# halixness/distributed-3d-diffusion-pytorch

Measured on AMD Instinct MI355X. Metric: train imgs/sec (whole node), SRN cars 64x64 bs128, higher is better.
Workload: dtype bf16; 1 GPU; model=XUNet ch128 ch_mult(1,2,2,4) 136.7M params (3DiM, reference xunet.py), global_batch=128, seq_len=4096, image_size=64, per_gpu_batch=128, micro_batch=128, hip_graph=False, parallelism=dp1, dist_backend=none, tuned_gemms=True, backend=hip

## Files before the change

### distributed_3d_diffusion_pytorch_amd/ops/_abi.py

```python
from __future__ import annotations

import ctypes as C

P = C.c_void_p
I = C.c_int
L = C.c_long
F = C.c_float
U64 = C.c_ulonglong
IP = C.POINTER(C.c_int)

SIGNATURES = {
    "d3d_gn_plan": [I, I, I, IP, IP],
    "d3d_gn_cfg": [I, I, I],
    "d3d_gn_cfg_small": [I, I],
    "d3d_gn_stats": [P, I, I, I, I, F, P, P, P, I, P],
    "d3d_gn_apply": [P, P, P, P, P, I, I, I, I, I, P],
    "d3d_gn_film": [P, P, P, P, P, P, I, I, I, I, F, U64, I, P, P],
    "d3d_gn_bwd": [I, P, P, P, P, P, P, I, I, I, I, F, U64, P, P, P, P, P, P, P, P],
    "d3d_ray_dir": [P, P, P, P, I, I, I, I, P],
    "d3d_border_fix": [P, P, I, I, I, I, I, I, I, P, P],
    "d3d_border_sums": [P, P, I, I, I, I, P],
    "d3d_gn_apply2": [I, P, P, P, P, P, P, P, I, I, I, I, F, F, U64, I, P, P, I, I, P, P],
    "d3d_set_words64": [P, I, C.c_longlong, C.c_longlong, C.c_longlong, P],
    "d3d_sgemm_jobs": [P, I, I, P],
    "d3d_gn_ab": [P, P, P, P, P, I, I, I, I, F, I, P],
    "d3d_gn_ab_silu": [P, P, P, I, I, I, P],
    "d3d_gn_img_cfg": [I],
    "d3d_gn_img_ok": [I, I, I],
    "d3d_gn_img_ok_n": [I, I, I, I],
    "d3d_gn_img_wide_cfg": [I, I],
    "d3d_gn_img_fwd": [I, P, P, P, P, P, P, I, I, I, I, F, F, U64, I, P, P, I, P, P],
    "d3d_gn_img_bwd": [I, P, P, P, P, P, P, I, I, I, I, F, U64, P, P, P, I, P, P, P, I, P, F, P, F, P],
    "d3d_gn_bwd2": [I, P, P, P, P, P, P, I, I, I, I, F, U64, P, P, P, P, P, P, P, I, I, P, P, P, I, P, F, P, F, P],
    "d3d_conv_s64_cfg": [I],
    "d3d_conv_hsm_cfg": [I],
    "d3d_gemm_small_k": [I],
    "d3d_gemm_mf": [I],
    "d3d_gemm_w8_waves": [I],
    "d3d_attn_bwd_cfg": [I],
    "d3d_attn_fwd_cfg": [I],
    "d3d_colsum_jobs": [P, I, P],
    "d3d_conv_halo_cfg": [I],
    "d3d_period_sum": [P, P, I, L, P],
    "d3d_silu": [P, P, L, P],
    "d3d_dsilu": [P, P, P, L, P],
    "d3d_avgpool2": [P, P, I, I, I, I, I, P],
    "d3d_upsample2": [P, P, I, I, I, I, I, P],
    "d3d_add_scale": [P, P, P, F, L, P],
    "d3d_set_words": [P, I, F, F, F, F, F, F, F, F, P],
    "d3d_add_scale_gn": [P, P, P, F, L, I, I, I, P, P],
    "d3d_sampler_step": [P, P, P, P, P, I, I, F, F, F, F, F, I, U64, I, P],
    "d3d_sampler_inputs": [P, P, I, I, P, P, U64, L, P, P, P],
    "d3d_sampler_step2": [P, P, P, I, I, P, P, U64, L, I, P],
    "d3d_sampler_solve": [P, P, P, P, I, I, P, P, U64, L, I, P],
    "d3d_randn_hash": [P, L, U64, L, P],
    "d3d_diffusion_fwd2": [P, I, I, U64, P, L, F, F, F, P, P, P, P, I, P],
    "d3d_diff_loss": [P, P, I, I, I, I, P, P, P, I, F, P],
    "d3d_diff_loss_bwd": [P, P, P, I, I, I, I, P, P, I, F, P],
    "d3d_adam": [P, P, P, P, P, L, F, F, F, F, F, F, F, F, P],
    "d3d_adam_dev": [P, P, P, P, P, L, P, P],
    "d3d_chansum": [P, P, P, P, I, I, I, I, P],
    "d3d_colsum": [P, L, I, P, P, P, I, P],
    "d3d_conv3_gn_ok": [I, I, I, I, I],
    "d3d_conv3_gn": [P, P, P, P, I, I, I, I, I, I, P, I, IP, P, P],
    "d3d_conv3": [P, P, P, P, P, P, I, I, I, I, I, I, I, I, I, I, I, F, I, I, P, I, P, I, IP, P, IP, P],
    "d3d_conv_plan": [I, I, I, I, I, I],
    "d3d_set_wgrad_impl": [I],
    "d3d_conv_wgrad_plan2": [I, I, I, I, I, I, IP, IP],
    "d3d_conv_wgrad_plan3": [I, I, I, I, I, I, I, I, I, IP, IP],
    "d3d_pack_weight": [P, P, I, I, I, I, I, I, P],
    "d3d_set_conv_impl": [I, P],
    "d3d_pack_all": [P, P, I, P],
    "d3d_conv_wgrad_cat": [P, P, P, I, P, P, P, I, I, I, I, I, I, P],
    "d3d_conv_wgrad_seg": [P, P, P, I, I, I, I, I, I, I, I, I, I, I, I, I, P, P, P, P],
    "d3d_wgrad_scatter": [P, I, I, I, I, P, I, I, P, P, P, P],
    "d3d_conv_wgrad3": [P, P, P, P, P, I, I, I, I, I, I, I, I, I, I, I, I, F, P],
    "d3d_ray_posenc": [P, P, P, P, P, P, P, P, I, I, I, P],
    "d3d_cond_prep": [P, P, P, I, C.c_double, C.c_double, P, P, P, P],
    "d3d_attn_fwd": [P, P, P, I, I, I, I, I, F, P],
    "d3d_adam_fused": [P, P, P, P, P, P, P, P, I, P, P, I, I, P],
    "d3d_mlp_ws": [I, I, I],
    "d3d_mlp_pe": [P, I, I, F, P, P],
    "d3d_mlp_mm": [P, P, I, I, I, I, I, I, P, P, P, P, P],
    "d3d_mlp_wgrad": [P, P, I, I, I, I, P, P, I, P],
    "d3d_gemm": [P, P, P, P, I, P, I, I, I, I, I, I, I, F, F, P, I, I, I, P],
    "d3d_gemm_cat": [P, P, P, I, P, P, I, I, I, I, I, F, F, P],
    "d3d_sgemm_strided": [P, P, P, I, I, I, I, L, L, L, L, L, L, L, L, L, F, F, P],
    "d3d_wgrad_tn_plan": [I, I, L, I, I],
    "d3d_wgrad_tn": [P, P, P, P, I, I, L, I, I, I, P],
    "d3d_wgrad_tn_tune": [I],
    "d3d_gemm_nt_ok": [I, I, I, I, I],
    "d3d_gemm_tune": [I, I, I],
    "d3d_gemm_nt": [P, P, P, P, P, I, I, I, I, I, I, I, F, F, P],
    "d3d_gemm_nt_gn": [P, P, P, P, P, I, I, I, I, I, I, I, F, F, P, I, I, P],
    "d3d_attn_bwd": [P, P, P, P, P, P, I, I, I, I, I, F, P],
    "d3d_attn_bwd_slabs": [I, I, I, I],
    "d3d_wgrad_group_cfg": [I, I, I],
    "d3d_wgrad_group_ok": [P],
    "d3d_wgrad_group_stages": [I],
    "d3d_wgrad_group_halo": [I, I, I],
    "d3d_wgrad_group_halo_big": [I, I],
    "d3d_wgrad_group_halo_pk": [I],
    "d3d_wgrad_group_engine": [P],
    "d3d_wgrad_group": [P, I, P, L, P],
    "d3d_wgrad_group_plan": [P, I, IP, IP, C.POINTER(C.c_long)],
    "d3d_loss_rows_parts": [I],
    "d3d_diff_loss_rows": [P, P, I, I, I, I, P, P, P],
    "d3d_loss_bins": [P, I, P, P, I, I, I, C.c_double, C.c_double, C.c_double, P],
    "d3d_image_metrics": [P, P, I, I, I, I, I, C.POINTER(C.c_double), P, P, P],
}


def declare(lib: C.CDLL) -> None:
    for name, args in SIGNATURES.items():
        fn = getattr(lib, name, None)
        if fn is None:
            continue
        fn.argtypes = args
        fn.restype = C.c_long if name in RET_LONG else C.c_int


RET_LONG = {"d3d_mlp_ws", "d3d_wgrad_group"}
```

### distributed_3d_diffusion_pytorch_amd/ops/csrc/conv.hip

```cpp
#include "common.h"
#include <stdlib.h>

#include <algorithm>

D3D_API int d3d_colsum(const float* in, long R, int Cc, float* part, float* out, float* out_odd, int accumulate,
                       hipStream_t st);

typedef __attribute__((ext_vector_type(4))) short s16x4;
typedef __attribute__((ext_vector_type(8))) short s16x8;
typedef __attribute__((address_space(3))) s16x4 lds_s16x4;

namespace {

template <int TAPS, bool TRANS>
__global__ void __launch_bounds__(256, 2)
conv_glds_k(const bf16* __restrict__ I, const bf16* __restrict__ Wp, const float* __restrict__ bias,
            const float* __restrict__ row_bias, const bf16* __restrict__ res, bf16* __restrict__ O,
            const bf16* __restrict__ zero16, int Nimg, int IH, int IW, int IC, int ICp, int OH, int OW, int OC,
            int ldo, int stride, float scale, int res_nmod, float* __restrict__ part, int korder) {
  constexpr int BM = 128, BN = 128, BKk = 64;
  constexpr int WM = 64, WN = 64, TM = 4, TN = 4;
  constexpr int STAGE = (BM + BN) * BKk;
  __shared__ __attribute__((aligned(16))) bf16 smem[2 * STAGE];
  typedef __attribute__((address_space(3))) void lds_void;
// ... 548 lines not shown
      for (int i = 0; i < TM; ++i)
#pragma unroll
        for (int j = 0; j < TN; ++j)
          acc[i][j] = __builtin_amdgcn_mfma_f32_16x16x32_bf16(af[i], bfr[j], acc[i][j], 0, 0, 0);
    }
    __builtin_amdgcn_s_setprio(0);
    asm volatile("s_waitcnt vmcnt(0) lgkmcnt(0)" ::: "memory");
    __builtin_amdgcn_s_barrier();
  }

  constexpr int NH = WN / 64;
  float gs[TM][NH], gq[TM][NH];
#pragma unroll
  for (int i = 0; i < TM; ++i)
#pragma unroll
    for (int h = 0; h < NH; ++h) gs[i][h] = gq[i][h] = 0.f;
  float cb[TM][4];
#pragma unroll
  for (int i = 0; i < TM; ++i) {
    const int co = m0 + wm * WM + i * 16 + fq * 4;
#pragma unroll
    for (int e = 0; e < 4; ++e) cb[i][e] = (bias && co + e < OC) ? bias[co + e] : 0.f;
  }
#pragma unroll
  for (int j = 0; j < TN; ++j) {
    const long pix = n0 + wn * WN + j * 16 + fr;
    if (pix >= Mpix) continue;
    const int img = (int)(pix / OHW);
    const long rpix = res_nmod > 0 ? (long)(img % res_nmod) * OHW + (pix - (long)img * OHW) : pix;
#pragma unroll
    for (int i = 0; i < TM; ++i) {
      const int co = m0 + wm * WM + i * 16 + fq * 4;
      if (co >= OC) continue;
      float v[4];
#pragma unroll
      for (int e = 0; e < 4; ++e) {
        const int cc = co + e < OC ? co + e : OC - 1;
        float t = acc[i][j][e] + cb[i][e];
        if (row_bias) t += row_bias[(long)img * OC + cc];
        v[e] = t;
      }
      bf16* dst = O + pix * ldo + co;
      if (co + 3 < OC && vec_out) {
        if constexpr (RES) {
          if (res) {
#pragma unroll
            for (int e = 0; e < 4; ++e) v[e] += (float)rres[i][j][e];
          }
        }
        bf16x4 o4;
#pragma unroll
        for (int e = 0; e < 4; ++e) {
          o4[e] = (bf16)(v[e] * scale);
          const float y = (float)o4[e];
          gs[i][j / 4] += y;
          gq[i][j / 4] += y * y;
        }
        *reinterpret_cast<bf16x4*>(dst) = o4;
        if (O2) silu_store4(O2, dst - O, o4);
      } else {
        for (int e = 0; e < 4 && co + e < OC; ++e) {
          float t = v[e];
          if (res) t += (float)res[rpix * ldo + co + e];
          dst[e] = (bf16)(t * scale);
          if (O2) O2[(dst - O) + e] = (bf16)siluf_((float)dst[e]);
          const float y = (float)dst[e];
          gs[i][j / 4] += y;
          gq[i][j / 4] += y * y;
        }
      }
    }
  }
  if (gnp) gn_part_store<TM, NH>(gs, gq, lane, m0 + wm * WM, n0 + wn * WN, OC, gn_groups, OHW, Mpix, gnp);
}

constexpr int HALO_CH = 32;

template <int OWT, int BNT = 512>
struct HaloGeom {
  static constexpr int TR = BNT / OWT;
  static constexpr int HW2 = (OWT + 2 + 7) / 8 * 8;
  static constexpr int HP = (TR + 2) * HW2;
  static constexpr int HPW = (HP + 127) / 128;
  static constexpr int HBUF = HPW * 8 * 16 * HALO_CH;
  static constexpr int ABUF = 128 * HALO_CH;
};

__device__ __forceinline__ void halo_issue_a(bf16* sA, const bf16* Wp, int w_bytes, int aoff, int soff, int wave) {
  typedef __attribute__((address_space(3))) void lds_void;
  const __amdgpu_buffer_rsrc_t rW = __builtin_amdgcn_make_buffer_rsrc((void*)Wp, (short)0, w_bytes, 0x00020000);
  __builtin_amdgcn_raw_ptr_buffer_load_lds(rW, (lds_void*)(sA + wave * 16 * HALO_CH), 16, aoff, soff, 0, 0);
}

template <int HPW>
__device__ __forceinline__ void halo_issue_b(bf16* sH, const bf16* I, int in_bytes, const unsigned* hoff, int cbyte,
                                             int wave) {
  typedef __attribute__((address_space(3))) void lds_void;
  const __amdgpu_buffer_rsrc_t rI = __builtin_amdgcn_make_buffer_rsrc((void*)I, (short)0, in_bytes, 0x00020000);
#pragma unroll
  for (int k = 0; k < HPW; ++k)
    __builtin_amdgcn_raw_ptr_buffer_load_lds(rI, (lds_void*)(sH + (wave + 8 * k) * 16 * HALO_CH), 16,
                                             hoff[k] + (unsigned)cbyte, 0, 0, 0);
}

template <int OWT, bool TRANS, int BNT = 512, bool RES = true, bool P2 = false, bool GNA = false>
__global__ void __launch_bounds__(512, 1)
conv_halo_k(const bf16* __restrict__ I, const bf16* __restrict__ Wp, const float* __restrict__ bias,
            const float* __restrict__ row_bias, const bf16* __restrict__ res, bf16* __restrict__ O, int in_bytes,
            int w_bytes, int Nimg, int OH, int IC, int ICp, int OC, float scale, int res_nmod,
            float* __restrict__ gnp, int gn_groups, bf16* __restrict__ O2, const float* __restrict__ gab) {
  static_assert(!GNA || (!P2 && !TRANS), "GroupNorm staging: forward, single-tap schedule");
  __shared__ __attribute__((aligned(16))) float sG[GNA ? 2 * 512 : 4];
  typedef HaloGeom<OWT, BNT> Gm;
  constexpr int BM = 128, BN = BNT, WM = 64, WN = BN / 4, TM = 4, TN = WN / 16;
  __shared__ __attribute__((aligned(16))) bf16 smem[2 * Gm::HBUF + (P2 ? 8 : 4) * Gm::ABUF];
  bf16* const sH = smem;
  bf16* const sAr = smem + 2 * Gm::HBUF;

  const int tid = threadIdx.x, lane = tid & 63;
  const int wave = __builtin_amdgcn_readfirstlane(tid >> 6);
  const int wm = wave >> 2, wn = wave & 3;
  const int OW = OWT, IH = OH, IW = OW;
  const int tiles = Nimg * (OH / Gm::TR);
  int bid = blockIdx.x;
  {
    int q = tiles / 8, r = tiles % 8, xcd = bid % 8;
    bid = (xcd < r ? xcd * (q + 1) : r * (q + 1) + (xcd - r) * q) + bid / 8;
  }
  const int img = bid / (OH / Gm::TR);
  const int r0 = (bid - img * (OH / Gm::TR)) * Gm::TR;
  const long n0 = ((long)img * OH + r0) * OW;
  const long Mpix = (long)Nimg * OH * OW;
  const int m0 = blockIdx.y * BM;
  const int Kp = 9 * ICp;

  const int arow = wave * 16 + (lane >> 2);
  const int aoff = ((m0 + arow) * Kp + (((lane & 3) ^ ((arow >> 1) & 2)) << 3)) * 2;
  unsigned hoff[Gm::HPW];
#pragma unroll
  for (int k = 0; k < Gm::HPW; ++k) {
    const int fi = (wave + 8 * k) * 16 + (lane >> 2);
    const int hr = fi / Gm::HW2, hc = fi - hr * Gm::HW2;
    const int ih = r0 - 1 + hr, iw = hc - 1;
    const bool ok = fi < Gm::HP && ih >= 0 && ih < IH && iw >= 0 && iw < IW;
    const int q = (lane & 3) ^ ((fi >> 1) & 2);
    const unsigned o = (unsigned)((((img * IH + (ok ? ih : 0)) * IW + (ok ? iw : 0)) * IC + q * 8) * 2);
    hoff[k] = ok ? o : 0x80000000u;
  }
  const int gnq = (lane & 3) ^ ((lane >> 3) & 2);
  auto gn_apply = [&](bf16* hb, int c) {
    if constexpr (GNA) {
      int lo = lane * 8 + wave * 16 * HALO_CH, to = (c * HALO_CH + gnq * 8) * 2;
      asm volatile("" : "+v"(lo), "+v"(to));
      const f32x4* t = reinterpret_cast<const f32x4*>(sG + to);
#pragma unroll
      for (int k = 0; k < Gm::HPW; ++k) {
        const bool ok = hoff[k] != 0x80000000u;
        bf16x2* q = reinterpret_cast<bf16x2*>(hb + lo + 8 * k * 16 * HALO_CH);
#pragma unroll
        for (int h = 0; h < 4; ++h) {
          const f32x4 a = t[h];
          const bf16x2 v = q[h];
          bf16x2 o;
          o[0] = (bf16)siluf_(__builtin_fmaf((float)v[0], a[0], a[1]));
          o[1] = (bf16)siluf_(__builtin_fmaf((float)v[1], a[2], a[3]));
          q[h] = ok ? o : v;
          __builtin_amdgcn_sched_barrier(0);
        }
      }
      asm volatile("s_waitcnt lgkmcnt(0)" ::: "memory");
    }
  };

  const int NCH = IC / HALO_CH, S = 9 * NCH;
  auto a_soff = [&](int s) {
    const int ss = s < S ? s : S - 1;
    const int c = ss / 9, t = ss - c * 9;
    return (t * ICp + c * HALO_CH) * 2;
  };

  f32x4 acc[TM][TN];
#pragma unroll
  for (int i = 0; i < TM; ++i)
#pragma unroll
    for (int j = 0; j < TN; ++j) acc[i][j] = f32x4{0.f, 0.f, 0.f, 0.f};

  const int fr = lane & 15, fq = lane >> 4;
  int hp0[TN];
#pragma unroll
  for (int j = 0; j < TN; ++j) {
    const int p = wn * WN + j * 16 + fr;
    hp0[j] = (p / OWT) * Gm::HW2 + (p % OWT);
  }
  const int OHW = OH * OW;
  if (RES && res) {
#pragma unroll
    for (int j = 0; j < TN; ++j) {
      const long pix = n0 + wn * WN + j * 16 + fr;
      const long rpix = res_nmod > 0 ? (long)(img % res_nmod) * OHW + (pix - (long)img * OHW) : pix;
#pragma unroll
      for (int i = 0; i < TM; ++i) {
        const int co = m0 + wm * WM + i * 16 + fq * 4;
        const bf16x4 r4 = co < OC ? *reinterpret_cast<const bf16x4*>(res + rpix * OC + co) : bf16x4{};
#pragma unroll
        for (int e = 0; e < 4; ++e) acc[i][j][e] = (float)r4[e];
      }
    }
  }

  if constexpr (P2) {
  halo_issue_b<Gm::HPW>(sH, I, in_bytes, hoff, 0, wave);
#pragma unroll
  for (int k = 0; k < 4; ++k) halo_issue_a(sAr + k * Gm::ABUF, Wp, w_bytes, aoff, a_soff(k), wave);
  int bo[3][TN], ao[TM];
#pragma unroll
  for (int kw = 0; kw < 3; ++kw)
#pragma unroll
    for (int j = 0; j < TN; ++j) {
      const int hp = hp0[j] + kw;
      bo[kw][j] = hp * HALO_CH + ((fq ^ ((hp >> 1) & 2)) << 3);
    }
#pragma unroll
  for (int i = 0; i < TM; ++i) {
    const int row = wm * WM + i * 16 + fr;
    ao[i] = row * HALO_CH + ((fq ^ ((row >> 1) & 2)) << 3);
  }
  auto step = [&](int s, int t, const bf16* hb) {
    const bf16* a = sAr + (s & 7) * Gm::ABUF;
    const int kh = TRANS ? 2 - t / 3 : t / 3, kw = TRANS ? 2 - t % 3 : t % 3;
    bf16x8 af[TM], bfr[TN];
#pragma unroll
    for (int j = 0; j < TN; ++j) bfr[j] = *reinterpret_cast<const bf16x8*>(hb + kh * Gm::HW2 * HALO_CH + bo[kw][j]);
#pragma unroll
    for (int i = 0; i < TM; ++i) af[i] = *reinterpret_cast<const bf16x8*>(a + ao[i]);
#pragma unroll
    for (int i = 0; i < TM; ++i)
#pragma unroll
      for (int j = 0; j < TN; ++j)
        acc[i][j] = __builtin_amdgcn_mfma_f32_16x16x32_bf16(af[i], bfr[j], acc[i][j], 0, 0, 0);
  };
  for (int c2 = 0; c2 < NCH; c2 += 2) {
    const int S0 = c2 * 9;
#pragma unroll
    for (int pp = 0; pp < 9; ++pp) {
      if (pp == 1 || pp == 2 || pp == 6 || pp == 7) {
        asm volatile("s_waitcnt vmcnt(%0)" ::"n"(2 + Gm::HPW) : "memory");
      } else {
        asm volatile("s_waitcnt vmcnt(2)" ::: "memory");
      }
      __builtin_amdgcn_s_barrier();
      const int s0 = S0 + 2 * pp;
      halo_issue_a(sAr + ((s0 + 4) & 7) * Gm::ABUF, Wp, w_bytes, aoff, a_soff(s0 + 4), wave);
      halo_issue_a(sAr + ((s0 + 5) & 7) * Gm::ABUF, Wp, w_bytes, aoff, a_soff(s0 + 5), wave);
      if (pp == 0 || pp == 5) {
        const int cn0 = c2 + (pp == 0 ? 1 : 2), cn = cn0 < NCH ? cn0 : NCH - 1;
        halo_issue_b<Gm::HPW>(sH + (cn0 & 1) * Gm::HBUF, I, in_bytes, hoff, cn * HALO_CH * 2, wave);
      }
      __builtin_amdgcn_s_setprio(1);
      const int sr0 = 2 * pp, sr1 = 2 * pp + 1;
      step(S0 + sr0, sr0 % 9, sH + (sr0 / 9) * Gm::HBUF);
      step(S0 + sr1, sr1 % 9, sH + (sr1 / 9) * Gm::HBUF);
      __builtin_amdgcn_s_setprio(0);
    }
  }
  } else {
  float gt[GNA ? 2 : 1];
  if constexpr (GNA) {
#pragma unroll
    for (int i = 0; i < 2; ++i) {
      const int j = tid + 512 * i;
      gt[i] = j < 2 * IC ? gab[(long)img * IC * 2 + j] : 0.f;
    }
  }
  halo_issue_b<Gm::HPW>(sH, I, in_bytes, hoff, 0, wave);
  halo_issue_a(sAr, Wp, w_bytes, aoff, a_soff(0), wave);
  halo_issue_a(sAr + Gm::ABUF, Wp, w_bytes, aoff, a_soff(1), wave);
  halo_issue_a(sAr + 2 * Gm::ABUF, Wp, w_bytes, aoff, a_soff(2), wave);
  if constexpr (GNA) {
#pragma unroll
    for (int i = 0; i < 2; ++i) sG[tid + 512 * i] = gt[i];
  }
  asm volatile("s_waitcnt vmcnt(0)" ::: "memory");
  if constexpr (GNA) {
    asm volatile("s_waitcnt lgkmcnt(0)" ::: "memory");
    __builtin_amdgcn_s_barrier();
    gn_apply(sH, 0);
  }
  int bo[3][TN], ao[TM];
#pragma unroll
  for (int kw = 0; kw < 3; ++kw)
#pragma unroll
    for (int j = 0; j < TN; ++j) {
      const int hp = hp0[j] + kw;
      bo[kw][j] = hp * HALO_CH + ((fq ^ ((hp >> 1) & 2)) << 3);
    }
#pragma unroll
  for (int i = 0; i < TM; ++i) {
    const int row = wm * WM + i * 16 + fr;
    ao[i] = row * HALO_CH + ((fq ^ ((row >> 1) & 2)) << 3);
  }
  for (int c = 0; c < NCH; ++c) {
    const bf16* hb = sH + (c & 1) * Gm::HBUF;
#pragma unroll
    for (int t = 0; t < 9; ++t) {
      const int s = c * 9 + t;
      if (t >= 1 && t <= 3) {
        asm volatile("s_waitcnt vmcnt(%0)" ::"n"(2 + Gm::HPW) : "memory");
      } else {
        asm volatile("s_waitcnt vmcnt(2)" ::: "memory");
      }
      __builtin_amdgcn_s_barrier();
      halo_issue_a(sAr + ((s + 3) & 3) * Gm::ABUF, Wp, w_bytes, aoff, a_soff(s + 3), wave);
      if (t == 0) {
        const int cn = c + 1 < NCH ? c + 1 : NCH - 1;
        halo_issue_b<Gm::HPW>(sH + ((c + 1) & 1) * Gm::HBUF, I, in_bytes, hoff, cn * HALO_CH * 2, wave);
      }
      if (t == 4) gn_apply(sH + ((c + 1) & 1) * Gm::HBUF, c + 1 < NCH ? c + 1 : NCH - 1);
      const bf16* a = sAr + (s & 3) * Gm::ABUF;
      __builtin_amdgcn_s_setprio(1);
      bf16x8 af[TM], bfr[TN];
      const int kh = TRANS ? 2 - t / 3 : t / 3, kw = TRANS ? 2 - t % 3 : t % 3;
#pragma unroll
      for (int j = 0; j < TN; ++j) bfr[j] = *reinterpret_cast<const bf16x8*>(hb + kh * Gm::HW2 * HALO_CH + bo[kw][j]);
#pragma unroll
      for (int i = 0; i < TM; ++i) af[i] = *reinterpret_cast<const bf16x8*>(a + ao[i]);
#pragma unroll
      for (int i = 0; i < TM; ++i)
#pragma unroll
        for (int j = 0; j < TN; ++j)
          acc[i][j] = __builtin_amdgcn_mfma_f32_16x16x32_bf16(af[i], bfr[j], acc[i][j], 0, 0, 0);
      __builtin_amdgcn_s_setprio(0);
    }
  }
  }
  asm volatile("s_waitcnt vmcnt(0)" ::: "memory");

  constexpr int NH = WN / 64;
  float gs[TM][NH], gq[TM][NH];
#pragma unroll
  for (int i = 0; i < TM; ++i)
#pragma unroll
    for (int h = 0; h < NH; ++h) gs[i][h] = gq[i][h] = 0.f;
  float cb[TM][4];
#pragma unroll
  for (int i = 0; i < TM; ++i) {
    const int co = m0 + wm * WM + i * 16 + fq * 4;
#pragma unroll
    for (int e = 0; e < 4; ++e) {
      float t = 0.f;
      if (co + e < OC) {
        if (bias) t += bias[co + e];
        if (row_bias) t += row_bias[(long)img * OC + co + e];
      }
      cb[i][e] = t;
    }
  }
#ifdef D3D_HALO_EPI_DIRECT
  constexpr bool LEPI = false;
#else
  constexpr bool LEPI = true;
#endif
  static_assert(2 * Gm::HBUF + (P2 ? 8 : 4) * Gm::ABUF >= BN * 128, "output tile must fit the LDS");
  const bool lepi = LEPI && (OC % 8) == 0;
  bf16* const sT = smem;
  if (lepi) {
    asm volatile("s_waitcnt lgkmcnt(0)" ::: "memory");
    __builtin_amdgcn_s_barrier();
  }
#pragma unroll
  for (int j = 0; j < TN; ++j) {
    const long pix = n0 + wn * WN + j * 16 + fr;
    const int pl = wn * WN + j * 16 + fr;
#pragma unroll
    for (int i = 0; i < TM; ++i) {
      const int co = m0 + wm * WM + i * 16 + fq * 4;
      if (co >= OC) continue;
      float v[4];
#pragma unroll
      for (int e = 0; e < 4; ++e) v[e] = acc[i][j][e] + cb[i][e];
      bf16x4 o4;
#pragma unroll
      for (int e = 0; e < 4; ++e) {
        o4[e] = (bf16)(v[e] * scale);
        const float y = (float)o4[e];
        gs[i][j / 4] += y;
        gq[i][j / 4] += y * y;
      }
      if (lepi) {
        const int cl = wm * WM + i * 16 + fq * 4;
        *reinterpret_cast<bf16x4*>(sT + pl * 128 + (((cl >> 3) ^ (pl & 15)) << 3) + (cl & 4)) = o4;
      } else {
        *reinterpret_cast<bf16x4*>(O + pix * OC + co) = o4;
        if (O2) silu_store4(O2, pix * OC + co, o4);
      }
    }
  }
  if (gnp) gn_part_store<TM, NH>(gs, gq, lane, m0 + wm * WM, n0 + wn * WN, OC, gn_groups, OHW, Mpix, gnp);
  if (lepi) {
    asm volatile("s_waitcnt lgkmcnt(0)" ::: "memory");
    __builtin_amdgcn_s_barrier();
#pragma unroll 4
    for (int idx = tid; idx < BN * 16; idx += 512) {
      const int pl = idx >> 4, c = idx & 15;
      const int co = m0 + c * 8;
      if (co >= OC) continue;
      const bf16x8 v = *reinterpret_cast<const bf16x8*>(sT + pl * 128 + ((c ^ (pl & 15)) << 3));
      const long off = (n0 + pl) * OC + co;
      *reinterpret_cast<bf16x8*>(O + off) = v;
      if (O2) {
        bf16x8 s8;
#pragma unroll
        for (int e = 0; e < 8; ++e) s8[e] = (bf16)siluf_((float)v[e]);
        *reinterpret_cast<bf16x8*>(O2 + off) = s8;
      }
    }
  }
}

__global__ void conv_splitk_epi_k(const float* __restrict__ part, int nsplit, long Mpix, int OC, int OHW,
                                  const float* __restrict__ bias, const float* __restrict__ row_bias,
                                  const bf16* __restrict__ res, int res_nmod, bf16* __restrict__ O, int ldo,
                                  float scale, bf16* __restrict__ O2) {
  const long nv = Mpix * (OC / 4);
  const long slab = Mpix * OC;
  for (long v = blockIdx.x * (long)blockDim.x + threadIdx.x; v < nv; v += (long)gridDim.x * blockDim.x) {
    long pix = v / (OC / 4);
    int co = (int)(v % (OC / 4)) * 4;
    f32x4 a = *reinterpret_cast<const f32x4*>(part + pix * OC + co);
    for (int sp = 1; sp < nsplit; ++sp) a += *reinterpret_cast<const f32x4*>(part + sp * slab + pix * OC + co);
    int img = (int)(pix / OHW);
#pragma unroll
    for (int e = 0; e < 4; ++e) {
      float t = a[e] + (bias ? bias[co + e] : 0.f);
      if (row_bias) t += row_bias[(long)img * OC + co + e];
      a[e] = t;
    }
    if (res) {
      const long rpix = res_nmod > 0 ? (long)(img % res_nmod) * OHW + (pix - (long)img * OHW) : pix;
      bf16x4 r4 = *reinterpret_cast<const bf16x4*>(res + rpix * ldo + co);
#pragma unroll
      for (int e = 0; e < 4; ++e) a[e] += (float)r4[e];
    }
    bf16x4 o4;
#pragma unroll
    for (int e = 0; e < 4; ++e) o4[e] = (bf16)(a[e] * scale);
// ... 1004 lines not shown
__global__ void __launch_bounds__(256) pack_all_k(const PackDesc* __restrict__ descs,
                                                  const int* __restrict__ blk_desc) {
  __shared__ float tile[32 * 16 * 9];
  const PackDesc d = descs[blk_desc[blockIdx.x]];
  const int local = blockIdx.x - d.blk0, tid = threadIdx.x;
  const int ics = d.ICs ? d.ICs : d.IC;
  const int T = d.taps;
  if (d.mode == 2) {
    const int t0 = local * 2048 + tid * 8;
    if (t0 >= d.OC) return;
    bf16x8 o;
#pragma unroll
    for (int e = 0; e < 8; ++e) o[e] = (bf16)(t0 + e < d.OC ? d.src[t0 + e] : 0.f);
    if (t0 + 7 < d.OC && ((reinterpret_cast<uintptr_t>(d.dst + t0) & 15) == 0))
      *reinterpret_cast<bf16x8*>(d.dst + t0) = o;
    else
      for (int e = 0; e < 8 && t0 + e < d.OC; ++e) d.dst[t0 + e] = o[e];
    return;
  }
  if (d.mode == 0) {
    const int ncg = (d.ICp + 255) / 256;
    const int co = local / ncg, ci0 = (local % ncg) * 256;
    const int nci = min(256, d.ICp - ci0);
    for (int k = tid; k < 256 * T; k += 256) {
      const int ci = ci0 + k / T;
      tile[k] = (co < d.OC && ci < d.IC) ? d.src[((long)co * ics + ci) * T + k % T] : 0.f;
    }
    __syncthreads();
    for (int k = tid; k < T * (nci / 8); k += 256) {
      const int tap = k / (nci / 8), c8 = (k % (nci / 8)) * 8;
      bf16x8 o;
#pragma unroll
      for (int e = 0; e < 8; ++e) o[e] = (bf16)tile[(c8 + e) * T + tap];
      *reinterpret_cast<bf16x8*>(d.dst + ((long)co * T + tap) * d.ICp + ci0 + c8) = o;
    }
    return;
  }
  const int nct = (d.OCp + 31) / 32;
  const int co0 = (local % nct) * 32, ci0 = (local / nct) * 16;
  for (int k = tid; k < 32 * 16 * T; k += 256) {
    const int r = k / (16 * T), q = k % (16 * T);
    const int co = co0 + r, ci = ci0 + q / T;
    tile[k] = (co < d.OC && ci < d.IC) ? d.src[((long)co * ics + ci) * T + q % T] : 0.f;
  }
  __syncthreads();
  for (int k = tid; k < 16 * T * 4; k += 256) {
    const int c8 = (k & 3) * 8, rt = k >> 2;
    const int ci = rt / T, tap = rt % T;
    if (ci0 + ci >= d.ICp || co0 + c8 >= d.OCp) continue;
    bf16x8 o;
#pragma unroll
    for (int e = 0; e < 8; ++e) o[e] = (bf16)tile[(c8 + e) * 16 * T + ci * T + tap];
    *reinterpret_cast<bf16x8*>(d.dst + ((long)(ci0 + ci) * T + tap) * (d.ldd ? d.ldd : d.OCp) + co0 + c8) = o;
  }
}

}

D3D_API int d3d_pack_all(const void* descs, const int* blk_desc, int total_blocks, hipStream_t st) {
  if (total_blocks <= 0) return 0;
  hipLaunchKernelGGL(pack_all_k, dim3(total_blocks), dim3(256), 0, st, (const PackDesc*)descs, blk_desc);
  return (int)hipGetLastError();
}

static int g_s64 = 1;
extern "C" int d3d_conv_s64_try(const void* I, const void* Wp, const float* bias, const float* row_bias,
                                const void* res, void* O, int N, int IH, int IW, int IC, int ICp, int OH, int OW,
                                int OC, int ldo, int stride, int trans, float scale, int res_nmod, int taps,
                                float* gnp, int gn_groups, int* gn_done, hipStream_t st, void* O2);
extern "C" int d3d_conv_hsm_try(const void* I, const void* Wp, const float* bias, const float* row_bias,
                                const void* res, void* O, int N, int IH, int IW, int IC, int ICp, int OH, int OW,
                                int OC, int ldo, int stride, int trans, float scale, int res_nmod, int taps,
                                const float* gnp, const void* O2, hipStream_t st);
static const long g_s64_maxb = 160;
static bool s64_wanted(long Mpix, int OC, int ICp, int taps) {
  const long blocks128 = ((Mpix + 127) / 128) * ((OC + 127) / 128);
  const long blocks64 = ((Mpix + 63) / 64) * (OC / 64);
  return g_s64 && OC % 64 == 0 && (taps * ICp) % 64 == 0 && blocks128 <= g_s64_maxb && blocks64 >= 128;
}
static int g_halo_w32 = 1;
static int g_halo_w16 = 1;
static int g_halo_w32s = 1;
static int g_halo_p2 = 1;
D3D_API int d3d_conv_halo_cfg(int cfg) {
  g_halo_w32 = (cfg >> 2) & 1;
  g_halo_w16 = (cfg >> 3) & 1;
  g_halo_w32s = (cfg >> 4) & 1;
  g_halo_p2 = (cfg >> 5) & 1;
  return 0;
}

enum ConvImpl {
  CONV_BUFL = 3,
  CONV_W8 = 4,
  CONV_W8W = 6,
  CONV_W8N = 7,
  CONV_HALO = 8,
};
enum WgradImpl {
  WGRAD_REG = 0,
  WGRAD_BUFL = 5,
  WGRAD_W8 = 6,
};
static int g_conv_impl = CONV_HALO;
static int g_wgrad_impl = WGRAD_W8;
static const bf16* g_zero16 = nullptr;
static const int kConvKorder = 1;

D3D_API int d3d_set_wgrad_impl(int impl) {
  if (impl != WGRAD_REG && impl != WGRAD_BUFL && impl != WGRAD_W8) return (int)hipErrorInvalidValue;
  g_wgrad_impl = impl;
  return 0;
}

D3D_API int d3d_set_conv_impl(int impl, const void* zero16) {
  if (impl != CONV_BUFL && impl != CONV_W8 && impl != CONV_W8W && impl != CONV_W8N && impl != CONV_HALO)
    return (int)hipErrorInvalidValue;
  g_conv_impl = impl;
  if (zero16) g_zero16 = (const bf16*)zero16;
  return 0;
}

D3D_API int d3d_conv_plan(int N, int OH, int OW, int OC, int ICp, int taps) {
  constexpr int BM = 128, BN = 128;
  long Mpix = (long)N * OH * OW;
  long blocks = ((Mpix + BN - 1) / BN) * ((OC + BM - 1) / BM);
  int nk = taps * ICp / 64;
  static const int target = 512;
  if (blocks >= 384 || (OC & 3)) return 1;
  if (s64_wanted(Mpix, OC, ICp, taps)) return 1;
  long want = target / blocks;
  long maxs = nk / 6;
  if (want > maxs) want = maxs;
  if (want > 16) want = 16;
  return want < 2 ? 1 : (int)want;
}

D3D_API int d3d_conv3(const void* I, const void* Wp, const float* bias, const float* row_bias, const void* res,
                      void* O, int N, int IH, int IW, int IC, int ICp, int OH, int OW, int OC, int ldo, int stride,
                      int trans, float scale, int res_nmod, int taps, float* ws, int nsplit, float* gnp,
                      int gn_groups, int* gn_done, void* O2, int* silu_done, hipStream_t st) {
  long Mpix = (long)N * OH * OW;
  if (gn_done) *gn_done = 0;
  if (silu_done) *silu_done = 0;
  if (!silu_done) O2 = nullptr;
  {
    const long img_in = (long)IH * IW * IC * 2, img_out = (long)OH * OW * ldo * 2;
    const long lim = (1L << 31) - (1L << 20);
    if (N > 1 && ((long)N * img_in >= lim || (long)N * img_out >= lim)) {
      long per = lim / std::max(img_in, img_out);
      const int q = res_nmod > 0 ? res_nmod : 1;
      per = per / q * q;
      if (per >= 1) {
        const int parts_per_img = (OH * OW) % 64 == 0 ? OH * OW / 64 : 0;
        int all_gn = 1, all_silu = 1;
        for (int n0 = 0; n0 < N; n0 += (int)per) {
          const int nc = (int)std::min<long>(per, N - n0);
          int d = 0, ds = 0;
          const int rc = d3d_conv3((const char*)I + n0 * img_in, Wp, bias,
                                   row_bias ? row_bias + (long)n0 * OC : nullptr,
                                   res ? (res_nmod > 0 ? res : (const char*)res + n0 * img_out) : nullptr,
                                   (char*)O + n0 * img_out, nc, IH, IW, IC, ICp, OH, OW, OC, ldo, stride, trans, scale,
                                   res_nmod, taps, ws, nsplit,
                                   gnp ? gnp + (long)n0 * gn_groups * parts_per_img * 2 : nullptr, gn_groups,
                                   gn_done ? &d : nullptr, O2 ? (char*)O2 + n0 * img_out : nullptr,
                                   O2 ? &ds : nullptr, st);
          if (rc) return rc;
          all_gn &= d;
          all_silu &= ds;
        }
        if (gn_done) *gn_done = gnp ? all_gn : 0;
        if (silu_done) *silu_done = O2 ? all_silu : 0;
        return 0;
      }
    }
  }
  if (gnp) {
    const int Cg = gn_groups > 0 && OC % gn_groups == 0 ? OC / gn_groups : 0;
    const bool ok = (Cg == 4 || Cg == 8 || Cg == 16 || Cg == 32) && (OH * OW) % 64 == 0 && Mpix % 64 == 0 &&
                    ldo == OC;
    if (!ok) gnp = nullptr;
  }
  constexpr int BM = 128, BN = 128;
  if (nsplit < 1 || !ws) nsplit = 1;
  if (nsplit == 1 && s64_wanted(Mpix, OC, ICp, taps)) {
    const int rh = d3d_conv_hsm_try(I, Wp, bias, row_bias, res, O, N, IH, IW, IC, ICp, OH, OW, OC, ldo, stride, trans,
                                    scale, res_nmod, taps, gnp, O2, st);
    if (rh != 0) return rh < 0 ? -rh : 0;
    const int r = d3d_conv_s64_try(I, Wp, bias, row_bias, res, O, N, IH, IW, IC, ICp, OH, OW, OC, ldo, stride, trans,
                                   scale, res_nmod, taps, gnp, gn_groups, gn_done, st, O2);
    if (r > 0 && silu_done) *silu_done = O2 ? 1 : 0;
    if (r != 0) return r < 0 ? -r : 0;
  }
  dim3 grid((unsigned)((Mpix + BN - 1) / BN), (unsigned)((OC + BM - 1) / BM), (unsigned)nsplit);
  const long in_bytes = (long)N * IH * IW * IC * 2, w_bytes = (long)((OC + 127) / 128 * 128) * taps * ICp * 2;
  if (g_conv_impl == CONV_HALO && taps == 9 && stride == 1 && IW == OW && IH == OH && ldo == OC && IC % HALO_CH == 0 &&
      OC % 128 == 0 && (OW == 16 || OW == 32 || OW == 64 || OW == 128) && in_bytes < (1L << 31) &&
      w_bytes < (1L << 31)) {
    auto nblk = [&](int bn) { return OH % (bn / OW) ? 0L : (long)N * (OH / (bn / OW)) * (OC / 128); };
    if ((OW != 32 || g_halo_w32) && nblk(512) >= 256) {
      dim3 gh((unsigned)(N * (OH / (512 / OW))), (unsigned)(OC / 128), 1);
#define HALO3(OWv, TR, RS, P2v)                                                                                   \
  hipLaunchKernelGGL((conv_halo_k<OWv, TR, 512, RS, (P2v && OWv != 128)>), gh, dim3(512), 0, st, (const bf16*)I,  \
                     (const bf16*)Wp, bias, row_bias, (const bf16*)res, (bf16*)O, (int)in_bytes, (int)w_bytes, N, OH, \
                     IC, ICp, OC, scale, res_nmod, gnp, gn_groups, (bf16*)O2, (const float*)nullptr)
#define HALO(OWv, TR, RS)                                                                                          \
  do {                                                                                                            \
    if (g_halo_p2 && OWv != 128 && (IC / HALO_CH) % 2 == 0) HALO3(OWv, TR, RS, true);                             \
    else HALO3(OWv, TR, RS, false);                                                                               \
  } while (0)
      if (OW == 64) {
        if (trans) { if (res) HALO(64, true, true); else HALO(64, true, false); }
        else if (res) HALO(64, false, true); else HALO(64, false, false);
      } else if (OW == 32) {
        if (trans) { if (res) HALO(32, true, true); else HALO(32, true, false); }
        else if (res) HALO(32, false, true); else HALO(32, false, false);
      } else {
        if (trans) { if (res) HALO(128, true, true); else HALO(128, true, false); }
        else if (res) HALO(128, false, true); else HALO(128, false, false);
      }
#undef HALO
#undef HALO3
      if (gn_done && gnp) *gn_done = 1;
      if (silu_done && O2) *silu_done = 1;
      return (int)hipGetLastError();
    }
    if (((OW == 16 && g_halo_w16) || (OW == 32 && g_halo_w32s)) && nblk(256) >= 256) {
      dim3 gh((unsigned)(N * (OH / (256 / OW))), (unsigned)(OC / 128), 1);
#define HALOS(OWv, TR, RS)                                                                                         \
  hipLaunchKernelGGL((conv_halo_k<OWv, TR, 256, RS>), gh, dim3(512), 0, st, (const bf16*)I,                        \
                     (const bf16*)Wp, bias, row_bias, (const bf16*)res, (bf16*)O, (int)in_bytes, (int)w_bytes, N, OH, \
                     IC, ICp, OC, scale, res_nmod, gnp, gn_groups, (bf16*)O2, (const float*)nullptr)
      if (OW == 16) {
        if (trans) { if (res) HALOS(16, true, true); else HALOS(16, true, false); }
        else if (res) HALOS(16, false, true); else HALOS(16, false, false);
      } else {
        if (trans) { if (res) HALOS(32, true, true); else HALOS(32, true, false); }
        else if (res) HALOS(32, false, true); else HALOS(32, false, false);
      }
#undef HALOS
      if (gn_done && gnp) *gn_done = 1;
      if (silu_done && O2) *silu_done = 1;
      return (int)hipGetLastError();
    }
  }
  if (g_conv_impl >= CONV_W8 && (!trans || stride == 1) && in_bytes < (1L << 31) && w_bytes < (1L << 31) && OC >= 64) {
    const int bm = (OC % 256 == 0 || OC > 384) ? 256 : 128;
    const bool wide = bm == 128 && g_conv_impl >= CONV_W8W;
    int bn = wide ? 512 : 256;
    long ptiles = (Mpix + bn - 1) / bn;
    long blocks = ptiles * ((OC + bm - 1) / bm);
    if (g_conv_impl == CONV_W8N && bm == 256 && blocks < 256 && ((Mpix + 127) / 128) * ((OC + 255) / 256) >= 256) {
      bn = 128;
      ptiles = (Mpix + bn - 1) / bn;
      blocks = ptiles * ((OC + bm - 1) / bm);
    }
    if ((bm == 256 || wide) && blocks >= 256) {
      dim3 g8((unsigned)ptiles, (unsigned)((OC + bm - 1) / bm), 1);
#define W8R(TP, TR, BMv, BNv, RS)                                                                                \
  hipLaunchKernelGGL((conv_w8_k<TP, TR, BMv, BNv, RS>), g8, dim3(512), 0, st, (const bf16*)I, (const bf16*)Wp, bias, \
                     row_bias, (const bf16*)res, (bf16*)O, (int)in_bytes, (int)w_bytes, N, IH, IW, IC, ICp, OH, OW, \
                     OC, ldo, stride, scale, res_nmod, kConvKorder, gnp, gn_groups, (bf16*)O2)
#define W8(TP, TR, BMv, BNv)                                                                                     \
  do {                                                                                                          \
    if (res) W8R(TP, TR, BMv, BNv, true); else W8R(TP, TR, BMv, BNv, false);                                     \
  } while (0)
      if (bn == 128) {
        if (taps == 9) {
          if (trans) W8(9, true, 256, 128); else W8(9, false, 256, 128);
        } else {
          if (trans) W8(1, true, 256, 128); else W8(1, false, 256, 128);
        }
      } else if (bm == 256) {
        if (taps == 9) {
          if (trans) W8(9, true, 256, 256); else W8(9, false, 256, 256);
        } else {
          if (trans) W8(1, true, 256, 256); else W8(1, false, 256, 256);
        }
      } else {
        if (taps == 9) {
          if (trans) W8(9, true, 128, 512); else W8(9, false, 128, 512);
        } else {
          if (trans) W8(1, true, 128, 512); else W8(1, false, 128, 512);
        }
      }
#undef W8
#undef W8R
      if (gn_done && gnp) *gn_done = 1;
      if (silu_done && O2) *silu_done = 1;
      return (int)hipGetLastError();
    }
  }
  if ((!trans || stride == 1) && in_bytes < (1L << 31) && w_bytes < (1L << 31)) {
    float* part = nsplit > 1 ? ws : nullptr;
#define BUFL(TP, TR)                                                                                             \
  hipLaunchKernelGGL((conv_bufl_k<TP, TR>), grid, dim3(256), 0, st, (const bf16*)I, (const bf16*)Wp, bias,        \
                     row_bias, (const bf16*)res, (bf16*)O, (int)in_bytes, (int)w_bytes, N, IH, IW, IC, ICp, OH, OW, \
                     OC, ldo, stride, scale, res_nmod, part, kConvKorder, part ? nullptr : gnp, gn_groups,         \
                     part ? nullptr : (bf16*)O2)
    if (taps == 9) {
      if (trans) BUFL(9, true); else BUFL(9, false);
    } else {
      if (trans) BUFL(1, true); else BUFL(1, false);
    }
#undef BUFL
    if (part && gnp && OC % 64 == 0) {
      hipLaunchKernelGGL(conv_splitk_epi_gn_k, dim3((unsigned)(Mpix / 64), (unsigned)(OC / 64)), dim3(256), 0, st,
                         part, nsplit, Mpix, OC, OH * OW, bias, row_bias, (const bf16*)res, res_nmod, (bf16*)O,
                         scale, gnp, gn_groups, (bf16*)O2);
      if (gn_done) *gn_done = 1;
    } else if (part) {
      long nv = Mpix * (OC / 4);
      long g = (nv + 255) / 256;
      if (g > 4096) g = 4096;
      hipLaunchKernelGGL(conv_splitk_epi_k, dim3((unsigned)g), dim3(256), 0, st, part, nsplit, Mpix, OC, OH * OW,
                         bias, row_bias, (const bf16*)res, res_nmod, (bf16*)O, ldo, scale, (bf16*)O2);
    } else if (gn_done && gnp) {
      *gn_done = 1;
    }
    if (silu_done && O2) *silu_done = 1;
    return (int)hipGetLastError();
  }
  if (!g_zero16) return (int)hipErrorInvalidValue;
  float* part = nsplit > 1 ? ws : nullptr;
#define GLDS(TP, TR)                                                                                             \
  hipLaunchKernelGGL((conv_glds_k<TP, TR>), grid, dim3(256), 0, st, (const bf16*)I, (const bf16*)Wp, bias,        \
                     row_bias, (const bf16*)res, (bf16*)O, g_zero16, N, IH, IW, IC, ICp, OH, OW, OC, ldo, stride, \
                     scale, res_nmod, part, kConvKorder)
  if (taps == 9) {
    if (trans) GLDS(9, true); else GLDS(9, false);
  } else {
    if (trans) GLDS(1, true); else GLDS(1, false);
  }
#undef GLDS
  if (part) {
    long nv = Mpix * (OC / 4);
    long g = (nv + 255) / 256;
    if (g > 4096) g = 4096;
    hipLaunchKernelGGL(conv_splitk_epi_k, dim3((unsigned)g), dim3(256), 0, st, part, nsplit, Mpix, OC, OH * OW,
                       bias, row_bias, (const bf16*)res, res_nmod, (bf16*)O, ldo, scale, (bf16*)nullptr);
  }
  return (int)hipGetLastError();
}

static int conv3_gn_shape(int N, int H, int W, int IC, int OC, int* tile) {
  const long in_bytes = (long)N * H * W * IC * 2, w_bytes = (long)((OC + 127) / 128 * 128) * 9 * ((IC + 63) / 64 * 64) * 2;
  if (g_conv_impl != CONV_HALO || IC % HALO_CH || OC % 128 || (W != 32 && W != 64) || in_bytes >= (1L << 31) ||
      w_bytes >= (1L << 31) || IC > 512)
    return 0;
  auto nblk = [&](int bn) { return H % (bn / W) ? 0L : (long)N * (H / (bn / W)) * (OC / 128); };
  if ((W != 32 || g_halo_w32) && nblk(512) >= 256) return 0;
  if (W == 32 && g_halo_w32s && nblk(256) >= 256) {
    *tile = 256;
    return 1;
  }
  return 0;
}

D3D_API int d3d_conv3_gn_ok(int N, int H, int W, int IC, int OC) {
  int t = 0;
  return conv3_gn_shape(N, H, W, IC, OC, &t);
}

D3D_API int d3d_conv3_gn(const void* I, const void* Wp, const float* bias, void* O, int N, int H, int W, int IC,
                         int ICp, int OC, float* gnp, int gn_groups, int* gn_done, const float* gab, hipStream_t st) {
  int tile = 0;
  if (gn_done) *gn_done = 0;
  if (!conv3_gn_shape(N, H, W, IC, OC, &tile) || ICp != (IC + 63) / 64 * 64) return -2;
  if (gnp) {
    const int Cg = gn_groups > 0 && OC % gn_groups == 0 ? OC / gn_groups : 0;
    if (!((Cg == 4 || Cg == 8 || Cg == 16 || Cg == 32) && (H * W) % 64 == 0)) gnp = nullptr;
  }
  const long in_bytes = (long)N * H * W * IC * 2, w_bytes = (long)((OC + 127) / 128 * 128) * 9 * ICp * 2;
  dim3 gh((unsigned)(N * (H / (tile / W))), (unsigned)(OC / 128), 1);
  hipLaunchKernelGGL((conv_halo_k<32, false, 256, false, false, true>), gh, dim3(512), 0, st, (const bf16*)I,
                     (const bf16*)Wp, bias, (const float*)nullptr, (const bf16*)nullptr, (bf16*)O, (int)in_bytes,
                     (int)w_bytes, N, H, IC, ICp, OC, 1.f, 0, gnp, gn_groups, (bf16*)nullptr, gab);
  if (gn_done && gnp) *gn_done = 1;
  return (int)hipGetLastError();
}

static void launch_reduce2(const float* ws, int OC, int IC, int taps, int splits, int accumulate, const float* bws,
                           int brows, float* dW, float* db, WSegs sg, bool want_bias, hipStream_t st,
                           float scale = 1.f) {
  if (taps == 9 && sg.n == 0) {
    const long base = (long)OC * ((IC + 63) / 64);
    const int tg = base >= 1024 ? 9 : (base * 3 >= 1024 ? 3 : 1);
    const int nblk_w = (int)(base * (9 / tg));
    const int nblk_b = want_bias ? (OC + 63) / 64 : 0;
#define R9(TGv) hipLaunchKernelGGL(wgrad_reduce9_k<TGv>, dim3(nblk_w + nblk_b), dim3(256), 0, st, ws, OC, IC, splits, \
                                  accumulate, bws, brows, dW, db, nblk_w, scale)
    if (tg == 9) R9(9); else if (tg == 3) R9(3); else R9(1);
#undef R9
    return;
  }
  int SL = 1;
  while (SL < splits && SL < 16) SL <<= 1;
  const long total = (long)OC * IC * taps;
  const int per = 4 * (256 / SL);
  const int nblk_w = (int)((total + per - 1) / per);
  const int nblk_b = want_bias ? (OC + per - 1) / per : 0;
  dim3 grid(nblk_w + nblk_b);
#define RL(S) hipLaunchKernelGGL(wgrad_reduce2_k<S>, grid, dim3(256), 0, st, ws, OC, IC, taps, splits, accumulate, \
                                 bws, brows, dW, db, sg, nblk_w, scale)
  switch (SL) {
    case 1: RL(1); break;
    case 2: RL(2); break;
    case 4: RL(4); break;
    case 8: RL(8); break;
    default: RL(16); break;
  }
#undef RL
}

static void launch_wgrad(const void* dY, const void* I, float* ws, int N, int IH, int IW, int IC, int OH, int OW,
                         int OC, int stride, int pps, int ncb, float* bws, int lw, int lh, int taps, dim3 grid,
                         hipStream_t st, const void* I2 = nullptr, int C1 = 0) {
  constexpr int BM = 128, BN = 128;
  const long in_elems = (long)N * IH * IW * IC;
  const bool wide_long = taps == 1 && (long)OC * IC >= (4L << 20) && pps > 16384;
  const bool fast = stride == 1 && lw >= 0 && IH == OH && IW == OW && IC % 128 == 0;
  if (g_wgrad_impl >= WGRAD_BUFL && !wide_long && (fast || in_elems * 2 < (1L << 31) - (1L << 20)) &&
      (long)pps * OC * 2 < (1L << 31)) {
    constexpr int PK = 32;
#define WB(TP, F)                                                                                                \
  hipLaunchKernelGGL((conv_wgrad_bufl_k<TP, PK, F>), grid, dim3(256), 0, st, (const bf16*)dY, (const bf16*)I, ws,   \
                     (long)N * IH * IW, N, IH, IW, IC, OH, OW, OC, stride, pps, ncb, bws, lw, lh, (const bf16*)I2, C1)
// ... 210 lines not shown
```

Baseline: 1110 examples/s.

## Run two halo-conv blocks per CU with a shorter weight ring and compact halo

Adds a 256-pixel halo conv variant with a 3-deep weight ring and a compacted halo buffer. Stray halo loads are redirected to a dummy LDS slot, so the block fits in half a CU's LDS and two blocks can be resident per CU. A new tile-selection helper picks this variant over the 512-pixel tile for 64-wide and some 32-wide layers when there are enough blocks, and it extends the 256 tile to W=64. The intent is more latency hiding through occupancy. The cost is a shallower prefetch pipeline, which may expose weight-load latency.

```diff
diff --git a/distributed_3d_diffusion_pytorch_amd/ops/_abi.py b/distributed_3d_diffusion_pytorch_amd/ops/_abi.py
--- a/distributed_3d_diffusion_pytorch_amd/ops/_abi.py
+++ b/distributed_3d_diffusion_pytorch_amd/ops/_abi.py
@@ -41,6 +41,9 @@
     "d3d_attn_fwd_cfg": [I],
     "d3d_colsum_jobs": [P, I, P],
     "d3d_conv_halo_cfg": [I],
+    "d3d_conv_halo_cus": [I],
+    "d3d_conv_halo_tile": [I, I, I, I, I, I, I],
+    "d3d_conv_halo_resident": [I, I, I],
     "d3d_period_sum": [P, P, I, L, P],
     "d3d_silu": [P, P, L, P],
     "d3d_dsilu": [P, P, P, L, P],
diff --git a/distributed_3d_diffusion_pytorch_amd/ops/csrc/conv.hip b/distributed_3d_diffusion_pytorch_amd/ops/csrc/conv.hip
--- a/distributed_3d_diffusion_pytorch_amd/ops/csrc/conv.hip
+++ b/distributed_3d_diffusion_pytorch_amd/ops/csrc/conv.hip
@@ -654,6 +654,7 @@
   static constexpr int HW2 = (OWT + 2 + 7) / 8 * 8;
   static constexpr int HP = (TR + 2) * HW2;
   static constexpr int HPW = (HP + 127) / 128;
+  static constexpr int HPC = (HP + 15) / 16;
   static constexpr int HBUF = HPW * 8 * 16 * HALO_CH;
   static constexpr int ABUF = 128 * HALO_CH;
 };
@@ -664,30 +665,40 @@
   __builtin_amdgcn_raw_ptr_buffer_load_lds(rW, (lds_void*)(sA + wave * 16 * HALO_CH), 16, aoff, soff, 0, 0);
 }
 
-template <int HPW>
+template <int HPW, int NP = HPW * 8>
 __device__ __forceinline__ void halo_issue_b(bf16* sH, const bf16* I, int in_bytes, const unsigned* hoff, int cbyte,
-                                             int wave) {
+                                             int wave, bf16* sD = nullptr) {
   typedef __attribute__((address_space(3))) void lds_void;
   const __amdgpu_buffer_rsrc_t rI = __builtin_amdgcn_make_buffer_rsrc((void*)I, (short)0, in_bytes, 0x00020000);
 #pragma unroll
-  for (int k = 0; k < HPW; ++k)
-    __builtin_amdgcn_raw_ptr_buffer_load_lds(rI, (lds_void*)(sH + (wave + 8 * k) * 16 * HALO_CH), 16,
-                                             hoff[k] + (unsigned)cbyte, 0, 0, 0);
-}
-
-template <int OWT, bool TRANS, int BNT = 512, bool RES = true, bool P2 = false, bool GNA = false>
-__global__ void __launch_bounds__(512, 1)
+  for (int k = 0; k < HPW; ++k) {
+    bf16* dst = sH + (wave + 8 * k) * 16 * HALO_CH;
+    if (8 * k + 7 >= NP) dst = wave + 8 * k < NP ? dst : sD;
+    __builtin_amdgcn_raw_ptr_buffer_load_lds(rI, (lds_void*)dst, 16, hoff[k] + (unsigned)cbyte, 0, 0, 0);
+  }
+}
+
+template <int OWT, bool TRANS, int BNT = 512, bool RES = true, bool P2 = false, bool GNA = false,
+          int RING = (P2 ? 8 : 4)>
+__global__ void __launch_bounds__(512, (BNT == 256 && RING < 4) ? 2 : 1)
 conv_halo_k(const bf16* __restrict__ I, const bf16* __restrict__ Wp, const float* __restrict__ bias,
             const float* __restrict__ row_bias, const bf16* __restrict__ res, bf16* __restrict__ O, int in_bytes,
             int w_bytes, int Nimg, int OH, int IC, int ICp, int OC, float scale, int res_nmod,
             float* __restrict__ gnp, int gn_groups, bf16* __restrict__ O2, const float* __restrict__ gab) {
   static_assert(!GNA || (!P2 && !TRANS), "GroupNorm staging: forward, single-tap schedule");
+  static_assert(P2 ? RING == 8 : (RING >= 2 && RING <= 4), "weight ring depth");
+  static_assert(RING >= 4 || (BNT == 256 && !GNA), "short rings: the two-resident 256-pixel tile only");
   __shared__ __attribute__((aligned(16))) float sG[GNA ? 2 * 512 : 4];
   typedef HaloGeom<OWT, BNT> Gm;
   constexpr int BM = 128, BN = BNT, WM = 64, WN = BN / 4, TM = 4, TN = WN / 16;
-  __shared__ __attribute__((aligned(16))) bf16 smem[2 * Gm::HBUF + (P2 ? 8 : 4) * Gm::ABUF];
+  constexpr bool CMP = RING == 3;
+  constexpr int NP = CMP ? Gm::HPC : Gm::HPW * 8, HBUF = NP * 16 * HALO_CH;
+  constexpr int SMEM = 2 * HBUF + RING * Gm::ABUF + (CMP ? 16 * HALO_CH : 0);
+  constexpr int D = RING - 1;
+  __shared__ __attribute__((aligned(16))) bf16 smem[SMEM];
   bf16* const sH = smem;
-  bf16* const sAr = smem + 2 * Gm::HBUF;
+  bf16* const sAr = smem + 2 * HBUF;
+  bf16* const sD = sAr + RING * Gm::ABUF;
 
   const int tid = threadIdx.x, lane = tid & 63;
   const int wave = __builtin_amdgcn_readfirstlane(tid >> 6);
@@ -844,10 +855,9 @@
       gt[i] = j < 2 * IC ? gab[(long)img * IC * 2 + j] : 0.f;
     }
   }
-  halo_issue_b<Gm::HPW>(sH, I, in_bytes, hoff, 0, wave);
-  halo_issue_a(sAr, Wp, w_bytes, aoff, a_soff(0), wave);
-  halo_issue_a(sAr + Gm::ABUF, Wp, w_bytes, aoff, a_soff(1), wave);
-  halo_issue_a(sAr + 2 * Gm::ABUF, Wp, w_bytes, aoff, a_soff(2), wave);
+  halo_issue_b<Gm::HPW, NP>(sH, I, in_bytes, hoff, 0, wave, sD);
+#pragma unroll
+  for (int k = 0; k < D; ++k) halo_issue_a(sAr + k * Gm::ABUF, Wp, w_bytes, aoff, a_soff(k), wave);
   if constexpr (GNA) {
 #pragma unroll
     for (int i = 0; i < 2; ++i) sG[tid + 512 * i] = gt[i];
@@ -872,23 +882,24 @@
     ao[i] = row * HALO_CH + ((fq ^ ((row >> 1) & 2)) << 3);
   }
   for (int c = 0; c < NCH; ++c) {
-    const bf16* hb = sH + (c & 1) * Gm::HBUF;
+    const bf16* hb = sH + (c & 1) * HBUF;
+    int sl = RING == 3 ? 0 : (c * 9) % RING;
 #pragma unroll
     for (int t = 0; t < 9; ++t) {
       const int s = c * 9 + t;
-      if (t >= 1 && t <= 3) {
-        asm volatile("s_waitcnt vmcnt(%0)" ::"n"(2 + Gm::HPW) : "memory");
+      if (t >= 1 && t <= D) {
+        asm volatile("s_waitcnt vmcnt(%0)" ::"n"(D - 1 + Gm::HPW) : "memory");
       } else {
-        asm volatile("s_waitcnt vmcnt(2)" ::: "memory");
+        asm volatile("s_waitcnt vmcnt(%0)" ::"n"(D - 1) : "memory");
       }
       __builtin_amdgcn_s_barrier();
-      halo_issue_a(sAr + ((s + 3) & 3) * Gm::ABUF, Wp, w_bytes, aoff, a_soff(s + 3), wave);
+      halo_issue_a(sAr + ((sl + t + D) % RING) * Gm::ABUF, Wp, w_bytes, aoff, a_soff(s + D), wave);
       if (t == 0) {
         const int cn = c + 1 < NCH ? c + 1 : NCH - 1;
-        halo_issue_b<Gm::HPW>(sH + ((c + 1) & 1) * Gm::HBUF, I, in_bytes, hoff, cn * HALO_CH * 2, wave);
-      }
-      if (t == 4) gn_apply(sH + ((c + 1) & 1) * Gm::HBUF, c + 1 < NCH ? c + 1 : NCH - 1);
-      const bf16* a = sAr + (s & 3) * Gm::ABUF;
+        halo_issue_b<Gm::HPW, NP>(sH + ((c + 1) & 1) * HBUF, I, in_bytes, hoff, cn * HALO_CH * 2, wave, sD);
+      }
+      if (t == D + 1) gn_apply(sH + ((c + 1) & 1) * HBUF, c + 1 < NCH ? c + 1 : NCH - 1);
+      const bf16* a = sAr + ((sl + t) % RING) * Gm::ABUF;
       __builtin_amdgcn_s_setprio(1);
       bf16x8 af[TM], bfr[TN];
       const int kh = TRANS ? 2 - t / 3 : t / 3, kw = TRANS ? 2 - t % 3 : t % 3;
@@ -932,7 +943,8 @@
 #else
   constexpr bool LEPI = true;
 #endif
-  static_assert(2 * Gm::HBUF + (P2 ? 8 : 4) * Gm::ABUF >= BN * 128, "output tile must fit the LDS");
+  static_assert(SMEM >= BN * 128, "output tile must fit the LDS");
+  static_assert(RING >= 4 || SMEM * 2 <= 81920, "two resident blocks: half a CU's LDS each");
   const bool lepi = LEPI && (OC % 8) == 0;
   bf16* const sT = smem;
   if (lepi) {
@@ -2103,12 +2115,44 @@
 static int g_halo_w16 = 1;
 static int g_halo_w32s = 1;
 static int g_halo_p2 = 1;
+#ifndef D3D_HALO_RING256
+#define D3D_HALO_RING256 3
+#endif
+static int g_halo_cfg = 125;
+static int g_halo_cus = 256;
 D3D_API int d3d_conv_halo_cfg(int cfg) {
+  g_halo_cfg = cfg;
   g_halo_w32 = (cfg >> 2) & 1;
   g_halo_w16 = (cfg >> 3) & 1;
   g_halo_w32s = (cfg >> 4) & 1;
   g_halo_p2 = (cfg >> 5) & 1;
   return 0;
+}
+D3D_API int d3d_conv_halo_cus(int cus) {
+  const int old = g_halo_cus;
+  if (cus > 0) g_halo_cus = cus;
+  return old;
+}
+
+static bool halo_2wg_wins(int W, int IC, long blocks, int cus) {
+  return W == 64 ? IC <= 128 : (IC <= 256 && blocks >= 4L * cus);
+}
+
+static int halo_tile(int N, int H, int W, int IC, int OC, int trans, int cfg, int cus) {
+  (void)trans;
+  if (IC % HALO_CH || OC % 128 || (W != 16 && W != 32 && W != 64 && W != 128)) return 0;
+  auto nblk = [&](int bn) { return H % (bn / W) ? 0L : (long)N * (H / (bn / W)) * (OC / 128); };
+  const bool w32 = (cfg >> 2) & 1, w16 = (cfg >> 3) & 1, w32s = (cfg >> 4) & 1, two = (cfg >> 6) & 1;
+  const bool all = (cfg >> 7) & 1;
+  const bool t512 = (W != 32 || w32) && nblk(512) >= cus;
+  if (two && t512 && (W == 64 || W == 32) && nblk(256) >= 2L * cus && (all || halo_2wg_wins(W, IC, nblk(256), cus)))
+    return 256;
+  if (t512) return 512;
+  if (((W == 16 && w16) || (W == 32 && w32s)) && nblk(256) >= cus) return 256;
+  return 0;
+}
+D3D_API int d3d_conv_halo_tile(int N, int H, int W, int IC, int OC, int trans, int cfg) {
+  return halo_tile(N, H, W, IC, OC, trans, cfg < 0 ? g_halo_cfg : cfg, g_halo_cus);
 }
 
 enum ConvImpl {
@@ -2218,8 +2262,8 @@
   if (g_conv_impl == CONV_HALO && taps == 9 && stride == 1 && IW == OW && IH == OH && ldo == OC && IC % HALO_CH == 0 &&
       OC % 128 == 0 && (OW == 16 || OW == 32 || OW == 64 || OW == 128) && in_bytes < (1L << 31) &&
       w_bytes < (1L << 31)) {
-    auto nblk = [&](int bn) { return OH % (bn / OW) ? 0L : (long)N * (OH / (bn / OW)) * (OC / 128); };
-    if ((OW != 32 || g_halo_w32) && nblk(512) >= 256) {
+    const int tile = halo_tile(N, OH, OW, IC, OC, trans, g_halo_cfg, g_halo_cus);
+    if (tile == 512) {
       dim3 gh((unsigned)(N * (OH / (512 / OW))), (unsigned)(OC / 128), 1);
 #define HALO3(OWv, TR, RS, P2v)                                                                                   \
   hipLaunchKernelGGL((conv_halo_k<OWv, TR, 512, RS, (P2v && OWv != 128)>), gh, dim3(512), 0, st, (const bf16*)I,  \
@@ -2246,18 +2290,22 @@
       if (silu_done && O2) *silu_done = 1;
       return (int)hipGetLastError();
     }
-    if (((OW == 16 && g_halo_w16) || (OW == 32 && g_halo_w32s)) && nblk(256) >= 256) {
+    if (tile == 256) {
       dim3 gh((unsigned)(N * (OH / (256 / OW))), (unsigned)(OC / 128), 1);
 #define HALOS(OWv, TR, RS)                                                                                         \
-  hipLaunchKernelGGL((conv_halo_k<OWv, TR, 256, RS>), gh, dim3(512), 0, st, (const bf16*)I,                        \
-                     (const bf16*)Wp, bias, row_bias, (const bf16*)res, (bf16*)O, (int)in_bytes, (int)w_bytes, N, OH, \
-                     IC, ICp, OC, scale, res_nmod, gnp, gn_groups, (bf16*)O2, (const float*)nullptr)
+  hipLaunchKernelGGL((conv_halo_k<OWv, TR, 256, RS, false, false, D3D_HALO_RING256>), gh, dim3(512), 0, st,        \
+                     (const bf16*)I, (const bf16*)Wp, bias, row_bias, (const bf16*)res, (bf16*)O, (int)in_bytes,   \
+                     (int)w_bytes, N, OH, IC, ICp, OC, scale, res_nmod, gnp, gn_groups, (bf16*)O2,                 \
+                     (const float*)nullptr)
       if (OW == 16) {
         if (trans) { if (res) HALOS(16, true, true); else HALOS(16, true, false); }
         else if (res) HALOS(16, false, true); else HALOS(16, false, false);
-      } else {
+      } else if (OW == 32) {
         if (trans) { if (res) HALOS(32, true, true); else HALOS(32, true, false); }
         else if (res) HALOS(32, false, true); else HALOS(32, false, false);
+      } else {
+        if (trans) { if (res) HALOS(64, true, true); else HALOS(64, true, false); }
+        else if (res) HALOS(64, false, true); else HALOS(64, false, false);
       }
 #undef HALOS
       if (gn_done && gnp) *gn_done = 1;
@@ -2364,6 +2412,24 @@
   return (int)hipGetLastError();
 }
 
+D3D_API int d3d_conv_halo_resident(int ow, int trans, int res) {
+  int n = 0;
+  hipError_t e = hipErrorInvalidValue;
+#define OCC(OWv, TR, RS) \
+  e = hipOccupancyMaxActiveBlocksPerMultiprocessor(&n, conv_halo_k<OWv, TR, 256, RS, false, false, D3D_HALO_RING256>, 512, 0)
+#define OCCW(OWv)                                                      \
+  do {                                                                 \
+    if (trans) { if (res) OCC(OWv, true, true); else OCC(OWv, true, false); } \
+    else if (res) OCC(OWv, false, true); else OCC(OWv, false, false);  \
+  } while (0)
+  if (ow == 16) OCCW(16);
+  else if (ow == 32) OCCW(32);
+  else if (ow == 64) OCCW(64);
+#undef OCCW
+#undef OCC
+  return e == hipSuccess ? n : -1;
+}
+
 static int conv3_gn_shape(int N, int H, int W, int IC, int OC, int* tile) {
   const long in_bytes = (long)N * H * W * IC * 2, w_bytes = (long)((OC + 127) / 128 * 128) * 9 * ((IC + 63) / 64 * 64) * 2;
   if (g_conv_impl != CONV_HALO || IC % HALO_CH || OC % 128 || (W != 32 && W != 64) || in_bytes >= (1L << 31) ||
```

Measured after the change: 1096 examples/s. 1.3% lower.
